# cheolwanpark/tiny-raytracer

Measured on AMD Instinct MI355X. Metric: Mray/s (primary+secondary), higher is better.
Workload: dtype f32; 1 GPU; cornell 2048x2048, depth 50, 256 spp per step (of 4096), streamed, reference-order BVH, seed 1; rays=160658711950, samples=22548578304, image_rows_per_gpu=2048, tuning=default, parallelism=single GPU, world_size=1, launched_by=plain

## Files before the change

### bindings/rust/tinyrt-sys/src/lib.rs

```rust
#![allow(non_camel_case_types)]

use std::os::raw::{c_char, c_int, c_void};

pub const TRT_ABI_VERSION: u32 = 4;

pub const TRT_OK: c_int = 0;
pub const TRT_ERR_INVALID_ARG: c_int = -1;
pub const TRT_ERR_DUPLICATE: c_int = -2;
pub const TRT_ERR_NOT_FOUND: c_int = -3;
pub const TRT_ERR_HIP: c_int = -4;
pub const TRT_ERR_NO_DEVICE: c_int = -5;
pub const TRT_ERR_OOM: c_int = -6;

pub const TRT_LAMBERTIAN: u32 = 0;
pub const TRT_METAL: u32 = 1;
pub const TRT_DIELECTRIC: u32 = 2;
pub const TRT_LIGHT: u32 = 3;

pub const TRT_BACKEND_MEGAKERNEL: u32 = 0;
pub const TRT_BACKEND_WAVEFRONT: u32 = 1;
pub const TRT_BACKEND_AUTO: u32 = 2;
pub const TRT_BACKEND_STREAMED: u32 = 3;

#[repr(C)]
// ... 601 lines not shown
    pub fn trt_denoise_color_default(out: *mut trt_denoise_color);
    pub fn trt_denoise_ex(input: *const trt_denoise_inputs, color: *const trt_denoise_color, width: u32, height: u32,
                          params: *const trt_denoise_params, out: *mut f32) -> c_int;
    pub fn trt_denoise_ex_device(d_in: *const trt_denoise_inputs, color: *const trt_denoise_color, width: u32, height: u32,
                                 params: *const trt_denoise_params, d_out: *mut f32, d_scratch: *mut c_void, scratch_bytes: u64,
                                 stream: *mut c_void) -> c_int;
    pub fn trt_tonemap_u8(accum: *const f32, npixels: u32, gamma: f32, rgb: *mut u8) -> c_int;
    pub fn trt_tonemap_u8_device(d_accum: *const f32, npixels: u32, gamma: f32, d_rgb: *mut u8, stream: *mut c_void) -> c_int;
    pub fn trt_streamed_chunk_spp(width: u32, rows: u32) -> u32;
    pub fn trt_kernel_timing_begin() -> c_int;
    pub fn trt_kernel_timing_end(total_ms: *mut f64, launches: *mut u32) -> c_int;

    pub fn trt_dominant_kernel(s: *const trt_scene, cam: *const trt_camera, p: *const trt_render_params) -> *const c_char;
    pub fn trt_flat_literal_compilations() -> u64;
    pub fn trt_flat_literal_diagnostic() -> *const c_char;

    pub fn trt_last_error() -> *const c_char;
    pub fn trt_device_count() -> c_int;
    pub fn trt_set_device(ordinal: c_int) -> c_int;
    pub fn trt_abi_version() -> u32;
}
```

### include/tinyrt.h

```cpp
#ifndef TINYRT_H
#define TINYRT_H

#include <stddef.h>
#include <stdint.h>

#ifdef __cplusplus
extern "C" {
#endif

#define TRT_ABI_VERSION 4

enum trt_status {
    TRT_OK = 0,
    TRT_ERR_INVALID_ARG = -1,
    TRT_ERR_DUPLICATE = -2,
    TRT_ERR_NOT_FOUND = -3,
    TRT_ERR_HIP = -4,
    TRT_ERR_NO_DEVICE = -5,
    TRT_ERR_OOM = -6
};

typedef struct { float x, y, z; } trt_vec3;
typedef struct { trt_vec3 origin, direction; } trt_ray;
typedef struct { uint32_t x, y; trt_ray ray; } trt_sample_point;
// ... 441 lines not shown
    uint32_t chunk_spp;
    uint32_t dual_walk;
    uint64_t workspace_bytes;
} trt_launch_plan;
int trt_streamed_launch_plan(const trt_scene *s, const trt_camera *cam, const trt_render_params *p, trt_launch_plan *out);

uint32_t trt_streamed_chunk_spp(uint32_t width, uint32_t rows);

int trt_kernel_timing_begin(void);
int trt_kernel_timing_end(double *total_ms, uint32_t *launches);

const char *trt_dominant_kernel(const trt_scene *s, const trt_camera *cam, const trt_render_params *p);

uint64_t trt_flat_literal_compilations(void);
const char *trt_flat_literal_diagnostic(void);

const char *trt_last_error(void);
int trt_device_count(void);
int trt_set_device(int ordinal);
uint32_t trt_abi_version(void);

#ifdef __cplusplus
}
#endif
#endif
```

### tiny-raytracer_amd/_lib.py

```python
import ctypes as C
import os
import subprocess

_HERE = os.path.dirname(os.path.abspath(__file__))
LIB_PATH = os.environ.get("TRT_LIB_PATH") or os.path.join(_HERE, "libtinyrt.so")
CSRC = os.path.join(_HERE, "csrc")

TRT_OK = 0
ABI_VERSION = 4
ERR_INVALID_ARG, ERR_DUPLICATE, ERR_NOT_FOUND, ERR_HIP, ERR_NO_DEVICE, ERR_OOM = -1, -2, -3, -4, -5, -6
LAMBERTIAN, METAL, DIELECTRIC, LIGHT = 0, 1, 2, 3
BACKEND_MEGAKERNEL, BACKEND_WAVEFRONT, BACKEND_AUTO, BACKEND_STREAMED = 0, 1, 2, 3


class Vec3(C.Structure):
    _fields_ = [("x", C.c_float), ("y", C.c_float), ("z", C.c_float)]

    def __init__(self, x=0.0, y=0.0, z=0.0):
        super().__init__(float(x), float(y), float(z))

    def tolist(self):
        return [self.x, self.y, self.z]


# ... 342 lines not shown
                                     C.c_uint64, C.c_void_p]),
    "trt_denoise_color_default": (None, [C.POINTER(DenoiseColor)]),
    "trt_denoise_ex": (C.c_int, [C.POINTER(DenoiseInputs), C.POINTER(DenoiseColor), C.c_uint32, C.c_uint32, C.POINTER(DenoiseParams), C.c_void_p]),
    "trt_denoise_ex_device": (C.c_int, [C.POINTER(DenoiseInputs), C.POINTER(DenoiseColor), C.c_uint32, C.c_uint32, C.POINTER(DenoiseParams),
                                        C.c_void_p, C.c_void_p, C.c_uint64, C.c_void_p]),
    "trt_streamed_chunk_spp": (C.c_uint32, [C.c_uint32, C.c_uint32]),
    "trt_tonemap_u8": (C.c_int, [C.c_void_p, C.c_uint32, C.c_float, C.c_void_p]),
    "trt_tonemap_u8_device": (C.c_int, [C.c_void_p, C.c_uint32, C.c_float, C.c_void_p, C.c_void_p]),
    "trt_dominant_kernel": (C.c_char_p, [C.c_void_p, C.POINTER(CameraPOD), C.POINTER(RenderParams)]),
    "trt_last_error": (C.c_char_p, []),
    "trt_device_count": (C.c_int, []),
    "trt_set_device": (C.c_int, [C.c_int]),
    "trt_abi_version": (C.c_uint32, []),
    "trt_flat_literal_compilations": (C.c_uint64, []),
    "trt_flat_literal_diagnostic": (C.c_char_p, []),
}


def build(force=False):
    if force and os.path.exists(LIB_PATH):
        os.remove(LIB_PATH)
    subprocess.run(["make", "-C", CSRC, "--no-print-directory"], check=True)
    return LIB_PATH


def _share_hip_runtime_with_torch():
    import importlib.util
    try:
        spec = importlib.util.find_spec("torch")
    except (ImportError, ValueError):
# ... 39 lines not shown
```

### tiny-raytracer_amd/csrc/capi.hip

```cpp
#include <hip/hip_runtime.h>

#include <math.h>
#include <stdio.h>
#include <stdlib.h>
#include <string.h>

#include <algorithm>
#include <memory>
#include <mutex>
#include <new>
#include <string>
#include <thread>
#include <vector>

#include "axis_quads.h"
#include "nearest_first.h"
#include "flat_reuse.h"
#include "host_stage.h"
#include "kernels.h"
#include "scene.h"
#include "scene_adopt.h"
#include "scene_cache.h"
#include "scene_query.h"
#include "stream_plan.h"

using namespace trt;

struct trt_world {
    World w;
};

namespace trt {
namespace {
std::mutex g_timing_mu;
bool g_timing_on = false;
unsigned g_timing_epoch = 0;
struct TimingPair { hipEvent_t begin, end; int device; };
// ... 25 lines not shown
    if (o.stream != stream || o.device != dev || o.epoch != epoch || hipEventCreate(&ev) != hipSuccess) {
        (void)hipGetLastError();
        (void)hipEventDestroy(o.ev);
        return;
    }
    if (hipEventRecord(ev, stream) != hipSuccess) { (void)hipGetLastError(); (void)hipEventDestroy(ev); (void)hipEventDestroy(o.ev); return; }
    std::lock_guard<std::mutex> lock(g_timing_mu);
    if (g_timing_on && g_timing_epoch == epoch) g_timing_pairs.push_back(TimingPair{o.ev, ev, dev});
    else { (void)hipEventDestroy(o.ev); (void)hipEventDestroy(ev); }
}
}

struct trt_scene {
    SceneHost host;
    FlatReuse flat_reuse{};
    std::vector<uint32_t> geo_index;
    SceneCache cache;
};

namespace {

thread_local std::string g_last_error;

int fail(int code, const std::string& msg) {
    g_last_error = msg;
    return code;
}
int fail_hip(hipError_t e, const char* what) {
    return fail(TRT_ERR_HIP, std::string(what) + ": " + hipGetErrorString(e));
}
// ... 1 lines not shown
    do {                                                     \
        hipError_t e_ = (call);                              \
        if (e_ != hipSuccess) return fail_hip(e_, #call);    \
    } while (0)

struct Defaults {
    trt_tuning tuning;
    trt_scene_options scene;
    bool flat_reuse = true;
    bool axis_quads = true;
    bool nearest_first = true;
    uint32_t flat_literal = 2;
    bool flat_literal_test_fail = false;
    uint32_t flat_literal_pairs = kLiteralIntervalPairs;
    uint32_t flat_literal_planes = kLiteralPlaneRegs;
};
const Defaults& defaults() {
    static const Defaults d = [] {
        Defaults x;
        x.tuning = tuning_builtin();
        x.scene = scene_options_builtin();
        auto env = [](const char* name) -> const char* { const char* e = getenv(name); return (e && *e) ? e : nullptr; };
        auto u32 = [&](const char* name, uint32_t& field) { if (const char* e = env(name)) field = (uint32_t)strtoul(e, nullptr, 10); };
        trt_tuning& t = x.tuning;
        u32("TRT_STREAM_MINW", t.stream_waves_per_simd); u32("TRT_BIG_THREADS", t.stream_big_threads); u32("TRT_STREAM_BATCH_SPP", t.stream_batch_spp);
        u32("TRT_RADIANCE_GB", t.radiance_gb); u32("TRT_LEAF_SLOTS", t.leaf_slots); u32("TRT_LDS_LEAF_STACK", t.lds_leaf_stack);
        u32("TRT_RAY_POOL", t.ray_pool); u32("TRT_STRAGGLERS", t.stragglers); u32("TRT_LDS_STRAGGLERS", t.lds_stragglers);
        u32("TRT_DUAL_WALK", t.dual_walk); u32("TRT_RUNTIME_WALK", t.runtime_walk); u32("TRT_XCD_REMAP", t.xcd_remap);
        u32("TRT_MINW", t.mega_waves_per_simd); u32("TRT_MEGA_THREADS", t.mega_threads); u32("TRT_MINW8", t.mega_global_waves8);
        u32("TRT_WF_MINW", t.wf_waves_per_simd); u32("TRT_WF_SERVE_MIN", t.wf_serve_min);
        trt_scene_options& o = x.scene;
        if (const char* e = env("TRT_CULL_PRUNE")) {
            const float v = (float)atof(e);
            if (v > 0.0f && v <= 1.0f) o.cull_prune = v;
        }
        if (const char* e = env("TRT_FLAT_WALK")) o.flat_walk = atoi(e) ? 1 : 0;
        if (const char* e = env("TRT_FLAT_REUSE")) x.flat_reuse = atoi(e) != 0;
        if (const char* e = env("TRT_AXIS_QUADS")) x.axis_quads = atoi(e) != 0;
        if (const char* e = env("TRT_NEAREST_FIRST")) x.nearest_first = atoi(e) != 0;
        if (const char* e = env("TRT_FLAT_LITERAL")) x.flat_literal = atoi(e) != 0 ? 1u : 0u;
        if (const char* e = env("TRT_FLAT_LITERAL_TEST_FAIL")) x.flat_literal_test_fail = atoi(e) != 0;
        if (const char* e = env("TRT_FLAT_LITERAL_PAIRS")) { const int v = atoi(e); if (v >= 3 && v <= 8) x.flat_literal_pairs = (uint32_t)v; }
        if (const char* e = env("TRT_FLAT_LITERAL_PLANES")) { const int v = atoi(e); if (v >= 0 && v <= 8 && *e >= '0' && *e <= '9') x.flat_literal_planes = (uint32_t)v; }
        if (const char* e = env("TRT_COMPACT_NODES")) o.compact_nodes = atoi(e) ? 1 : 0;
        if (const char* e = env("TRT_SCRATCH_CAP_MB")) o.scratch_cap_bytes = (uint64_t)strtoull(e, nullptr, 10) << 20;
        return x;
    }();
    return d;
}

[[maybe_unused]] const bool g_defaults_read_at_load = (defaults(), true);

int require_device() {
    int n = 0;
    hipError_t e = hipGetDeviceCount(&n);
    if (e != hipSuccess || n <= 0) {
        (void)hipGetLastError();
        return fail(TRT_ERR_NO_DEVICE, "no HIP device visible: libtinyrt has no CPU path, it needs a gfx950 GPU");
// ... 117 lines not shown
            s->cache.set_short_samples(dev, (rc == TRT_OK && samples < wanted) ? samples : 0u);
        }
        if (rc != TRT_OK) return rc;
        LiteralRequest lit;
        const SceneLayout& L = s->host.layout;
        if (streamed && defaults().flat_literal != 0u && L.flat_walk != 0u && L.n_leaves > 0u &&
            s->host.blob.size() >= 16u * ((size_t)L.off_leaf_list + 2u * (size_t)L.n_leaves)) {
            lit.slot = s->cache.literal_kernel(dev);
            lit.leaf_list = s->host.blob.data() + 16u * (size_t)L.off_leaf_list;
            lit.n_leaves = L.n_leaves;
            const uint64_t call_samples = (uint64_t)cam->width * rows * (ra.sample_end - ra.sample_begin);
            lit.wanted = defaults().flat_literal == 1u || call_samples >= kLiteralAutoSamples;
            lit.empty_source = defaults().flat_literal_test_fail;
            lit.interval_pairs = defaults().flat_reuse ? defaults().flat_literal_pairs : 3u;
            lit.plane_regs = defaults().flat_reuse ? defaults().flat_literal_planes : 0u;
        }
        const LiteralScope lit_scope(lit.slot ? &lit : nullptr);
        hipError_t le;
        if (streamed && d_moment2) {
            le = launch_moments ? launch_moments(sc, cd, ra, tn, ws->ptr, ws->bytes, d_accum, d_moment2, reinterpret_cast<unsigned long long*>(d_counters),
                                                 p->collect_stats != 0, stream)
                                : hipErrorInvalidDeviceFunction;
        } else if (streamed) {
            le = launch_streamed(sc, cd, ra, tn, ws->ptr, ws->bytes, d_accum, reinterpret_cast<unsigned long long*>(d_counters), p->collect_stats != 0, stream);
        } else {
            le = launch_wavefront(sc, cd, ra, tn, ws->ptr, d_accum, reinterpret_cast<unsigned long long*>(d_counters), p->collect_stats != 0, stream);
        }
        rc = s->cache.workspace_release(dev, ws, stream);
        if (le != hipSuccess) return fail_hip(le, streamed ? "launch_streamed" : "launch_wavefront");
        return rc;
// ... 5 lines not shown
void set_flat_reuse(trt_scene* s) {
    const SceneLayout& L = s->host.layout;
    const size_t end = 16u * ((size_t)L.off_leaf_list + 2u * (size_t)L.n_leaves);
    const bool have = L.flat_walk != 0u && L.n_leaves > 0u && s->host.blob.size() >= end;
    uint32_t m[3];
    flat_reuse_masks(have ? s->host.blob.data() + 16u * (size_t)L.off_leaf_list : nullptr, L.n_leaves, have && defaults().flat_reuse, m);
    const size_t qend = 16u * ((size_t)L.off_quad + 5u * (size_t)L.n_quads);
    const bool have_quads = have && L.n_quads > 0u && s->host.blob.size() >= qend;
    const uint32_t aq = axis_quads_flag(have_quads ? s->host.blob.data() + 16u * (size_t)L.off_quad : nullptr, L.n_quads, L.n_leaves, L.flat_walk != 0u,
                                        scene_mode(L) == 1, defaults().axis_quads);
    float planes[3];
    const uint32_t nf = nearest_first_flag(have ? s->host.blob.data() + 16u * (size_t)L.off_leaf_list : nullptr, L.n_leaves,
                                           have_quads ? s->host.blob.data() + 16u * (size_t)L.off_quad : nullptr, L.n_quads, L.n_spheres, aq,
                                           defaults().nearest_first, planes);
    s->flat_reuse = FlatReuse{m[0], m[1], m[2], aq, nf, planes[0], planes[1], planes[2]};
}

void set_geo_index(trt_scene* s) {
    const SceneLayout& L = s->host.layout;
    const std::vector<int32_t>& geo = s->host.reference.prim_geo;
    s->geo_index.assign((size_t)L.n_spheres + L.n_quads, 0xFFFFFFFFu);
    const size_t end = 16u * ((size_t)L.off_ref_nodes + 2u * (size_t)L.n_nodes);
    if (geo.size() < L.n_nodes || s->host.blob.size() < end) return;
    for (uint32_t i = 0; i < L.n_nodes; i++) {
        if (geo[i] < 0) continue;
        uint32_t link;
        memcpy(&link, s->host.blob.data() + 16u * ((size_t)L.off_ref_nodes + 2u * (size_t)i + 1u) + 12u, 4);
        const size_t slot = (size_t)(link & PRIM_INDEX_MASK) + ((link & PRIM_QUAD_BIT) ? L.n_spheres : 0u);
        if (!(link & NODE_INNER_BIT) && slot < s->geo_index.size()) s->geo_index[slot] = (uint32_t)geo[i];
    }
// ... 194 lines not shown
int trt_scene_get_cull_nodes(const trt_scene* s, float* bbox6, int32_t* prim, int32_t* skip, uint32_t cap) {
    if (!s || !bbox6 || !prim || !skip) return fail(TRT_ERR_INVALID_ARG, "null argument");
    return copy_nodes(s->host.culling, bbox6, prim, skip, cap);
}

int trt_scene_get_compact_nodes(const trt_scene* s, uint32_t* words4, uint32_t cap) {
    if (!s || !words4) return fail(TRT_ERR_INVALID_ARG, "null argument");
    const SceneLayout& L = s->host.layout;
    if (L.off_compact == 0u) return fail(TRT_ERR_NOT_FOUND, "scene has no compact node array (it is walked from LDS)");
    if (cap < L.n_cull_nodes) return fail(TRT_ERR_INVALID_ARG, "buffer too small");
    memcpy(words4, s->host.blob.data() + 16u * (size_t)L.off_compact, 16u * (size_t)L.n_cull_nodes);
    for (uint32_t i = 0; i < L.n_cull_nodes; i++)
        if (!(words4[4u * (size_t)i + 3u] & 0x80000000u)) words4[4u * (size_t)i + 3u] >>= 4;
    return TRT_OK;
}
int trt_scene_get_packed(const trt_scene* s, uint8_t* bytes, uint32_t cap) {
    if (!s || !bytes) return fail(TRT_ERR_INVALID_ARG, "null argument");
    const uint32_t n = s->host.layout.blob_bytes;
    if (cap < n) return fail(TRT_ERR_INVALID_ARG, "cap is smaller than the packed scene (trt_scene_info.device_bytes)");
    memcpy(bytes, s->host.blob.data(), n);
    return TRT_OK;
}
int trt_scene_emitters(const trt_scene* s, trt_emitter* out, uint32_t cap, uint32_t* count) {
    if (!s || !count) return fail(TRT_ERR_INVALID_ARG, "null argument");
    if (cap > 0u && !out) return fail(TRT_ERR_INVALID_ARG, "out is null");
    const SceneLayout& L = s->host.layout;
    const F4* const f4 = reinterpret_cast<const F4*>(s->host.blob.data());
    const uint32_t* const u32 = reinterpret_cast<const uint32_t*>(s->host.blob.data());
    try {
        std::vector<trt_emitter> lights;
// ... 431 lines not shown
```

### tiny-raytracer_amd/csrc/flat_literal_rtc.h

```cpp
#pragma once

#include <dlfcn.h>
#include <stdint.h>

#include <string>
#include <vector>

#include "flat_literal.h"

namespace trt {

struct RtcHeader { const char* name; const char* text; };
inline const std::vector<RtcHeader>& rtc_project_headers() {
    static const std::vector<RtcHeader> h = {
#include "rtc_headers.inc"
    };
    return h;
}
inline const std::vector<RtcHeader>& rtc_system_headers() {
    static const std::vector<RtcHeader> h = {
        {"hip/hip_runtime.h", "#pragma once\n"},
        {"stdint.h", "#pragma once\n"
                     "typedef signed char int8_t; typedef unsigned char uint8_t; typedef short int16_t; typedef unsigned short uint16_t;\n"
                     "typedef int int32_t; typedef unsigned int uint32_t; typedef long int64_t; typedef unsigned long uint64_t;\n"
// ... 36 lines not shown
        auto sym = [&](auto& fn, const char* name) { fn = reinterpret_cast<std::remove_reference_t<decltype(fn)>>(dlsym(h, name)); return fn != nullptr; };
        a.ok = sym(a.create, "hiprtcCreateProgram") && sym(a.destroy, "hiprtcDestroyProgram") && sym(a.add_name, "hiprtcAddNameExpression") &&
               sym(a.compile, "hiprtcCompileProgram") && sym(a.log_size, "hiprtcGetProgramLogSize") && sym(a.log, "hiprtcGetProgramLog") &&
               sym(a.lowered, "hiprtcGetLoweredName") && sym(a.code_size, "hiprtcGetCodeSize") && sym(a.code, "hiprtcGetCode");
        return a;
    }();
    return api;
}

struct FlatLiteralBuild {
    std::vector<char> code;
    std::string kernel;
    std::string log;
};

inline std::string flat_literal_source(const std::string& asm_text, uint32_t extra_operands = 0u) {
    return flat_literal_define("TRT_FLAT_LITERAL_ASM", asm_text) + "#define TRT_FLAT_LITERAL_EXTRA " + std::to_string(extra_operands) +
           "\n#include \"stream_pool.h\"\n";
}

inline bool flat_literal_compile(const std::string& source, int minw, const char* arch, const void* beside, FlatLiteralBuild& out) {
    const HiprtcApi& rtc = hiprtc_api(beside);
    if (!rtc.ok) { out.log = "hiprtc not found"; return false; }
    std::vector<const char*> names, texts;
    for (const auto* set : {&rtc_system_headers(), &rtc_project_headers()})
        for (const RtcHeader& h : *set) { names.push_back(h.name); texts.push_back(h.text); }
    HiprtcApi::Program prog = nullptr;
    if (rtc.create(&prog, source.c_str(), "stream_pool_literal.hip", (int)names.size(), texts.data(), names.data()) != 0) { out.log = "hiprtcCreateProgram failed"; return false; }
    const std::string expr = "&trt::stream_pool_kernel<1, false, " + std::to_string(minw) + ", 256, 2, true>";
    const std::string arch_opt = std::string("--offload-arch=") + arch;
    const char* opts[] = {arch_opt.c_str(), "-O3", "-std=c++17", "-ffp-contract=off", "-fno-fast-math", "-fno-slp-vectorize"};
    int rc = rtc.add_name(prog, expr.c_str());
    if (rc == 0) rc = rtc.compile(prog, (int)(sizeof(opts) / sizeof(opts[0])), opts);
// ... 15 lines not shown
```

### tiny-raytracer_amd/csrc/literal_kernel.h

```cpp
#pragma once

#include <stdint.h>

#include <condition_variable>
#include <mutex>

namespace trt {

struct LiteralKernel {
    enum State { UNTRIED, COMPILING, READY, FAILED };
    std::mutex mu;
    std::condition_variable cv;
    State state = UNTRIED;
    void* module = nullptr;
    void* function = nullptr;
    int minw = 0;
    void (*unload)(void* module) = nullptr;
    void release() {
        if (module && unload) unload(module);
        module = function = nullptr;
        state = UNTRIED;
    }
};

constexpr uint32_t kLiteralIntervalPairs = 8u, kLiteralPlaneRegs = 6u;

struct LiteralRequest {
    LiteralKernel* slot = nullptr;
    const void* leaf_list = nullptr;
    uint32_t n_leaves = 0;
    bool wanted = false;
    bool empty_source = false;
    uint32_t interval_pairs = kLiteralIntervalPairs;
    uint32_t plane_regs = kLiteralPlaneRegs;
};
inline thread_local const LiteralRequest* t_literal_request = nullptr;
class LiteralScope {
  public:
    explicit LiteralScope(const LiteralRequest* r) { t_literal_request = r; }
    LiteralScope(const LiteralScope&) = delete;
    ~LiteralScope() { t_literal_request = nullptr; }
};

constexpr uint64_t kLiteralAutoSamples = 1ull << 26;

}
```

### tiny-raytracer_amd/csrc/rt_path.h

```cpp
#pragma once

#include "axis_quads.h"
#include "nearest_first.h"
#include "kernels.h"
#include "rt_device.h"
#include "stream_plan.h"

namespace trt {

extern __shared__ float4 g_lds[];


template <int MODE>
struct SceneAcc {
    const float4* blob;
    SceneLayout L;
    TRT_DEV float4 f4(uint32_t idx) const { return MODE == MODE_LDS ? g_lds[idx] : blob[idx]; }
    TRT_DEV uint32_t u32(uint32_t idx) const {
        return MODE == MODE_LDS ? reinterpret_cast<const uint32_t*>(g_lds)[idx] : reinterpret_cast<const uint32_t*>(blob)[idx];
    }
    TRT_DEV void node(uint32_t i, float4& a, float4& b) const { a = f4(2u * i); b = f4(2u * i + 1u); }
    TRT_DEV void ref_node(uint32_t i, float4& a, float4& b) const { a = blob[L.off_ref_nodes + 2u * i]; b = blob[L.off_ref_nodes + 2u * i + 1u]; }
    TRT_DEV float4 sphere(uint32_t i) const { return f4(L.off_sphere + i); }
    TRT_DEV float4 quad(uint32_t plane, uint32_t i) const { return f4(L.off_quad + 5u * i + plane); }
    TRT_DEV float4 material(uint32_t i) const { return f4(L.off_material + i); }
// ... 112 lines not shown
        pass = slab_fast(na, nb, ray.o, tr.inv, kTMin, tr.t_best);
    } else {
        sc.ref_node(tr.i, na, nb);
        if (tr.fast) pass = slab_fast(na, nb, ray.o, tr.inv, kTMin, tr.t_best);
        else pass = slab_exact(na, nb, ray.o, tr.inv, kTMin, tr.t_best);
    }
    const uint32_t link = __float_as_uint(nb.w);
    const bool inner = (link & NODE_INNER_BIT) != 0u;
    tr.i = (pass && inner) ? (link & ~NODE_INNER_BIT) : __float_as_uint(nb.z);
    return (pass && !inner) ? link : PRIM_NONE;
}

template <int MODE, bool STATS, bool COLD = false>
TRT_DEV void trav_leaf(const SceneAcc<MODE>& sc, const Ray& ray, Trav& tr, uint32_t leaf, Counters<STATS>& ctr, uint32_t axis_quads = 0u) {
    const uint32_t idx = leaf & PRIM_INDEX_MASK;
    if (axis_quads != 0u && (leaf & PRIM_QUAD_BIT)) {
        if constexpr (STATS) ctr.quad_plane++;
        const float4 q0 = sc.quad(0, idx), q1 = sc.quad(1, idx), q2 = sc.quad(2, idx), q3 = sc.quad(3, idx);
        const V3 nrm = v3(q0.x, q0.y, q0.z);
        const float dir_norm = dot(ray.d, nrm);
        const float t = (q0.w - dot(ray.o, nrm)) / dir_norm;
        const bool in_range = (kTMin <= t) & (t < tr.t_best);
        if constexpr (STATS) { if (in_range) ctr.quad_inside++; }
        const V3 p = ray_at(ray, t) - v3(q1.x, q1.y, q1.z);
        const float planar_x = q2.w * dot(p, v3(q2.x, q2.y, q2.z));
        const float planar_y = q2.w * dot(p, v3(q3.x, q3.y, q3.z));
        if (in_range & (0.0f <= planar_x) & (planar_x < 1.0f) & (0.0f <= planar_y) & (planar_y < 1.0f)) {
            tr.t_best = t;
            tr.prim_best = leaf;
        }
    } else if (leaf & PRIM_QUAD_BIT) {
        if constexpr (STATS) ctr.quad_plane++;
        const float4 q0 = sc.quad(0, idx), q1 = sc.quad(1, idx), q2 = sc.quad(2, idx), q3 = sc.quad(3, idx), q4 = sc.quad(4, idx);
        const V3 nrm = v3(q0.x, q0.y, q0.z);
        const float dir_norm = dot(ray.d, nrm);
        const float t = (q0.w - dot(ray.o, nrm)) / dir_norm;
        const bool in_range = (kTMin <= t) & (t < tr.t_best);
        if constexpr (STATS) { if (in_range) ctr.quad_inside++; }
        const V3 p = ray_at(ray, t) - v3(q1.x, q1.y, q1.z);
        const V3 vv = v3(q2.x, q2.y, q2.z), ww = v3(q2.w, q3.x, q3.y), uu = v3(q3.z, q3.w, q4.x);
        const float planar_x = dot(cross(p, vv), ww);
        const float planar_y = dot(cross(uu, p), ww);
        if (in_range & (0.0f <= planar_x) & (planar_x < 1.0f) & (0.0f <= planar_y) & (planar_y < 1.0f)) {
            tr.t_best = t;
            tr.prim_best = leaf;
        }
// ... 690 lines not shown
template <int MODE, bool STATS, int WALK, bool ANY = false>
TRT_DEV bool closest_hit_resume(const SceneAcc<MODE>& sc, const Ray& ray, Trav& tr, Counters<STATS>& ctr, uint32_t leaf_slots, float2* lds_stack,
                                const float4* __restrict__ leaf_list, const uint4* __restrict__ nodes16, uint32_t stragglers, uint32_t entered) {
    static_assert(WALK == WALK_COMPACT || WALK == WALK_LDS_STACK, "only the per-lane tree walks with an LDS leaf stack can be left and resumed");
    if (__builtin_expect(!tr.ref, 1)) {
        if constexpr (WALK == WALK_COMPACT) return walk_compact<MODE, STATS, ANY>(sc, nodes16, leaf_list, ray, tr, ctr, lds_stack, leaf_slots, stragglers, entered);
        else return walk_fast_lds<MODE, STATS, ANY>(sc, ray, tr, ctr, lds_stack, leaf_slots, stragglers, entered);
    }
    closest_hit_ref<MODE, STATS, ANY>(sc, ray, tr, ctr);
    return true;
}

template <int MODE>
TRT_DEV uint32_t prim_material(const SceneAcc<MODE>& sc, uint32_t prim) {
    const uint32_t idx = prim & PRIM_INDEX_MASK;
    return (prim & PRIM_QUAD_BIT) ? __float_as_uint(sc.quad(1, idx).w) : sc.sphere_material(idx);
}

struct Path {
    Ray ray;
    V3 color, atten;
    uint32_t remain;
    Rng rng;
};

constexpr uint32_t SHADE_KIND_MISS = 0xFFFFFFFFu;
struct ShadeInfo {
    bool hide_light;
    uint32_t kind;
    V3 normal;
};
template <int MODE, bool STATS, bool LAZY, bool INFO>
TRT_DEV bool shade_body(const SceneAcc<MODE>& sc, Path& p, uint32_t prim, float t, V3 background, Counters<STATS>& ctr, ShadeInfo* info) {
    if (prim == PRIM_NONE) {
        p.color = (LAZY ? v3(0.0f, 0.0f, 0.0f) : p.color) + p.atten * background;
        if constexpr (INFO) info->kind = SHADE_KIND_MISS;
        return true;
    }
    if constexpr (STATS) ctr.shade++;
    const uint32_t idx = prim & PRIM_INDEX_MASK;
    V3 point = ray_at(p.ray, t);
    V3 normal;
    bool front_face;
    uint32_t mat;
    if (prim & PRIM_QUAD_BIT) {
        float4 q0 = sc.quad(0, idx), q1 = sc.quad(1, idx), q4 = sc.quad(4, idx);
        front_face = dot(p.ray.d, v3(q0.x, q0.y, q0.z)) < 0.0f;
        V3 nu = v3(q4.y, q4.z, q4.w);
        normal = front_face ? nu : -nu;
        mat = __float_as_uint(q1.w);
    } else {
        float4 sp = sc.sphere(idx);
        V3 outward = point - v3(sp.x, sp.y, sp.z);
        front_face = dot(p.ray.d, outward) < 0.0f;
        V3 nu = normalized(outward);
        normal = front_face ? nu : -nu;
        mat = sc.sphere_material(idx);
    }
    const float4 m = sc.material(mat);
    const uint32_t kind = sc.material_kind(mat);
// ... 41 lines not shown
    } else {
        return true;
    }
    p.atten = p.atten * albedo;
    p.ray = ray_new(point, dir);
    p.remain -= 1u;
    return p.remain == 0u;
}
template <int MODE, bool STATS, bool LAZY = false>
TRT_DEV bool shade_hit(const SceneAcc<MODE>& sc, Path& p, uint32_t prim, float t, V3 background, Counters<STATS>& ctr) {
    return shade_body<MODE, STATS, LAZY, false>(sc, p, prim, t, background, ctr, nullptr);
}
template <int MODE, bool STATS>
TRT_DEV bool shade_hit_info(const SceneAcc<MODE>& sc, Path& p, uint32_t prim, float t, V3 background, Counters<STATS>& ctr, ShadeInfo& info) {
    return shade_body<MODE, STATS, false, true>(sc, p, prim, t, background, ctr, &info);
}

TRT_DEV Ray primary_ray(const CameraDev& cam, uint32_t x, uint32_t y, Rng& rng) {
    const float nu = (float)x + rng_random(rng);
    const float nv = (float)y + rng_random(rng);
    float u, v;
    pixel_uv(cam.width, cam.height, nu, nv, u, v);
    float px, py;
    random_in_unit_disk(rng, px, py);
    V3 pos = v3(cam.pos[0], cam.pos[1], cam.pos[2]);
    V3 du = v3(cam.du[0], cam.du[1], cam.du[2]), dv = v3(cam.dv[0], cam.dv[1], cam.dv[2]);
    V3 origin = (pos + px * du) + py * dv;
    V3 ul = v3(cam.upper_left[0], cam.upper_left[1], cam.upper_left[2]);
    V3 hor = v3(cam.horizontal[0], cam.horizontal[1], cam.horizontal[2]);
    V3 ver = v3(cam.vertical[0], cam.vertical[1], cam.vertical[2]);
// ... 66 lines not shown
```

### tiny-raytracer_amd/csrc/stream_pool.h

```cpp
#pragma once

#include "kernels.h"
#include "rt_path.h"
#include "stream_plan.h"
#include "wave_run.h"

namespace trt {

struct StreamKernargs {
    SceneDev scd; CameraDev cam; RenderArgs ra;
    float* colors; uint32_t* batch_counter; unsigned long long* counters;
    uint32_t tiles_x, n_tiles, n_batches, batch_spp;
    const float4* leaf_list; const uint4* nodes16;
};
struct StreamTileArgs { uint32_t tiles_x, n_tiles, n_batches, batch_spp; };
template <class T>
TRT_DEV T kernarg_reload(size_t offset) {
    static_assert(sizeof(T) % 4 == 0, "whole words");
    typedef const __attribute__((address_space(4))) uint32_t* WordPtr;
    WordPtr w = (WordPtr)__builtin_amdgcn_kernarg_segment_ptr() + offset / 4;
    asm volatile("" : "+s"(w));
    uint32_t words[sizeof(T) / 4];
#pragma unroll
    for (uint32_t i = 0; i < sizeof(T) / 4; i++) words[i] = w[i];
// ... 104 lines not shown
            if constexpr (kResumable) {
                Trav tr = trav_begin<MODE, WALK == WALK_COMPACT>(sc, p.ray, false);
                if (walking) trav_unpark(leaf_stack, tr); else n_rays++;
                const uint32_t entered = (uint32_t)__builtin_popcountll(__builtin_amdgcn_ballot_w64(true));
                walking = !closest_hit_resume<MODE, STATS, WALK>(sc, p.ray, tr, ctr, ra.leaf_slots, leaf_stack, leaf_list, nodes16, ra.stragglers, entered);
                if (!walking) {
                    if (shade_hit<MODE, STATS, LAZY>(sc, p, tr.prim_best, tr.t_best, background, ctr)) {
                        radiance_store(kernarg_reload<float*>(offsetof(StreamKernargs, colors)), out_idx, p.color);
                        has_path = false;
                    }
                }
            } else {
                n_rays++;
                float t;
                const uint32_t prim = closest_hit<MODE, STATS, WALK>(sc, p.ray, STATS && ra.ref_tree != 0u, t, ctr, ra.leaf_slots, leaf_stack, leaf_list, nodes16, flat_reuse);
                if (shade_hit<MODE, STATS, LAZY>(sc, p, prim, t, background, ctr)) {
                    radiance_store(kernarg_reload<float*>(offsetof(StreamKernargs, colors)), out_idx, p.color);
                    has_path = false;
                }
            }
        }
        TRT_CLK(ctr, 3);
    }
    flush_counters<STATS>(counters, n_samples, n_rays, ctr);
}

}
```

### tiny-raytracer_amd/csrc/streamed.hip

```cpp
#include <mutex>
#include <string>

#include "flat_literal_rtc.h"
#include "host_stage.h"
#include "kernels.h"
#include "literal_kernel.h"
#include "rt_path.h"
#include "stream_plan.h"
#include "stream_pool.h"
#include "wave_run.h"

namespace trt {

template <int MODE, bool STATS, int MINW = 1, int THREADS = 256, int WALK = WALK_RUNTIME, bool LAZY = false>
__global__ __launch_bounds__(THREADS, MINW) void stream_sample_kernel(SceneDev scd, CameraDev cam, RenderArgs ra,
                                                                             float* __restrict__ colors,
                                                                             uint32_t* __restrict__ batch_counter,
                                                                             unsigned long long* __restrict__ counters,
                                                                             uint32_t tiles_x, uint32_t n_tiles, uint32_t n_batches, uint32_t batch_spp,
                                                                             const float4* __restrict__ leaf_list,
                                                                             const uint4* __restrict__ nodes16) {
    stage_scene_to_lds<MODE>(scd);
    const FlatReuse flat_reuse = axis_quads_to_lds<MODE, STATS, WALK>(scd, ra.flat_reuse);
    const SceneAcc<MODE> sc{scd.blob, scd.L};
// ... 315 lines not shown
#define TRT_FN_POOL(MODE, STATS, MINW, THREADS, WALK, LAZY) reinterpret_cast<const void*>(&stream_pool_kernel<MODE, STATS, MINW, THREADS, WALK, LAZY>),
#define TRT_FN_SAMPLE(MODE, STATS, MINW, THREADS, WALK, LAZY) reinterpret_cast<const void*>(&stream_sample_kernel<MODE, STATS, MINW, THREADS, WALK, LAZY>),
#define TRT_FN_DUAL(MINW) reinterpret_cast<const void*>(&stream_dual_kernel<MINW, 256>),
const void* const kStreamKernelFns[] = {
    TRT_STREAM_SPECIALISED(TRT_FN_POOL, TRT_FN_SAMPLE, TRT_FN_DUAL)
    TRT_STREAM_GENERAL(TRT_FN_POOL, TRT_FN_SAMPLE, TRT_FN_DUAL)
};
#undef TRT_FN_POOL
#undef TRT_FN_SAMPLE
#undef TRT_FN_DUAL
static_assert(sizeof(kStreamKernelFns) / sizeof(kStreamKernelFns[0]) == kStreamKernelCount, "one address per shape row");

std::mutex g_literal_mu;
unsigned long long g_literal_compilations = 0;
std::string g_literal_diagnostic;
thread_local std::string t_literal_diagnostic_copy;

void literal_unload(void* module) {
    (void)hipModuleUnload(static_cast<hipModule_t>(module));
    (void)hipGetLastError();
}

bool literal_build(LiteralKernel& slot, const LiteralRequest& rq, const FlatReuse& reuse, int minw, std::string& why) {
    {
        std::lock_guard<std::mutex> lock(g_literal_mu);
        g_literal_compilations++;
    }
    int dev = 0;
    hipDeviceProp_t prop;
    if (hipGetDevice(&dev) != hipSuccess || hipGetDeviceProperties(&prop, dev) != hipSuccess) { (void)hipGetLastError(); why = "no device properties"; return false; }
    std::string arch(prop.gcnArchName);
    arch = arch.substr(0, arch.find(':'));
    const uint32_t masks[3] = {reuse.x, reuse.y, reuse.z};
    std::string text, source;
    if (!rq.empty_source) {
        FlatCacheStats cache;
        if (!flat_literal_cached_asm(rq.leaf_list, rq.n_leaves, masks, rq.interval_pairs, rq.plane_regs, text, cache)) { why = "leaf list refused"; return false; }
        source = flat_literal_source(text, cache.extra_operands);
    }
    FlatLiteralBuild built;
    if (!flat_literal_compile(source, minw, arch.c_str(), reinterpret_cast<const void*>(&hipModuleLoadData), built)) { why = "hiprtc: " + built.log; return false; }
    hipModule_t mod = nullptr;
    hipFunction_t fn = nullptr;
    hipError_t e = hipModuleLoadData(&mod, built.code.data());
    if (e == hipSuccess) e = hipModuleGetFunction(&fn, mod, built.kernel.c_str());
    if (e != hipSuccess) {
        (void)hipGetLastError();
        if (mod) (void)hipModuleUnload(mod);
        why = std::string("module load: ") + hipGetErrorString(e);
        return false;
    }
    slot.module = mod; slot.function = fn; slot.minw = minw; slot.unload = &literal_unload;
    return true;
}

hipFunction_t literal_kernel_for(const StreamLaunchPlan& pl, const RenderArgs& ra, bool stats) {
    const LiteralRequest* rq = t_literal_request;
#ifdef TRT_PHASE_CLOCK
    return nullptr;
#endif
    if (!kAsmBoxLoop) return nullptr;
    if (!rq || !rq->slot || stats || !pl.specialised || !pl.pool || pl.dual || pl.walk != WALK_FLAT || pl.mode != MODE_LDS || ra.ref_tree ||
        pl.kernel_walk != WALK_FLAT || pl.threads != 256 || pl.lds_bytes > 48u * 1024u || rq->n_leaves > kFlatLiteralMaxLeaves) return nullptr;
    LiteralKernel& slot = *rq->slot;
    std::unique_lock<std::mutex> lock(slot.mu);
    while (slot.state == LiteralKernel::COMPILING) slot.cv.wait(lock);
    if (slot.state == LiteralKernel::UNTRIED && rq->wanted) {
        slot.state = LiteralKernel::COMPILING;
        lock.unlock();
        std::string why;
        const bool ok = literal_build(slot, *rq, ra.flat_reuse, pl.kernel_minw, why);
        if (!ok) {
            std::lock_guard<std::mutex> g(g_literal_mu);
            g_literal_diagnostic = "lock-step kernel not compiled for its scene, the built-in kernel runs: " + why;
        }
        lock.lock();
        slot.state = ok ? LiteralKernel::READY : LiteralKernel::FAILED;
        slot.cv.notify_all();
    }
    if (slot.state != LiteralKernel::READY || slot.minw != pl.kernel_minw) return nullptr;
    return static_cast<hipFunction_t>(slot.function);
}

}

static hipError_t launch_streamed_folds(const SceneDev& sc, const CameraDev& cam, const RenderArgs& ra_all, const trt_tuning& tn, void* workspace, size_t workspace_bytes,
                                        float* d_accum, float* d_moment2, unsigned long long* d_counters, bool stats, hipStream_t stream) {
    if (ra_all.rows_local == 0 || cam.width == 0) return hipSuccess;
    uint32_t* batch_counter = static_cast<uint32_t*>(workspace);
    float* colors = reinterpret_cast<float*>(static_cast<char*>(workspace) + kWorkspaceHeader);
    const uint32_t samples_all = ra_all.sample_end - ra_all.sample_begin;
    uint32_t chunk_full = streamed_chunk_spp(cam.width, ra_all.rows_local, tn.radiance_gb);
    const uint32_t granted = streamed_chunk_that_fits(cam.width, ra_all.rows_local, workspace_bytes);
    if (granted == 0u) return hipErrorInvalidValue;
    if (chunk_full > granted) chunk_full = granted;
// ... 88 lines not shown

int trt_variance_device(const float* d_accum, const float* d_moment2, uint32_t npixels, uint32_t samples_per_pixel, float* d_variance, void* stream) {
    if (npixels && (!d_accum || !d_moment2 || !d_variance)) return trt::query_fail(TRT_ERR_INVALID_ARG, "null argument");
    if (npixels == 0u) return TRT_OK;
    const int rc = trt::query_require_device();
    if (rc != TRT_OK) return rc;
    const hipError_t e = trt::launch_variance(d_accum, d_moment2, npixels, samples_per_pixel, d_variance, static_cast<hipStream_t>(stream));
    if (e != hipSuccess) return trt::query_fail_hip(e, "variance launch");
    return TRT_OK;
}

uint64_t trt_flat_literal_compilations(void) {
    std::lock_guard<std::mutex> lock(trt::g_literal_mu);
    return trt::g_literal_compilations;
}
const char* trt_flat_literal_diagnostic(void) {
    std::lock_guard<std::mutex> lock(trt::g_literal_mu);
    trt::t_literal_diagnostic_copy = trt::g_literal_diagnostic;
    return trt::t_literal_diagnostic_copy.c_str();
}

int trt_variance(const float* accum, const float* moment2, uint32_t npixels, uint32_t samples_per_pixel, float* variance) {
    return trt::host_form([&]() -> int {
        if (npixels && (!accum || !moment2 || !variance)) return trt::query_fail(TRT_ERR_INVALID_ARG, "null argument");
        if (npixels == 0u) return TRT_OK;
        const int rc = trt::query_require_device();
        if (rc != TRT_OK) return rc;
        const size_t frame = (size_t)npixels * 12u;
        trt::HostStage st("variance buffers");
        const size_t r_s = st.reserve(frame), r_m = st.reserve(frame), r_v = st.reserve((size_t)npixels * 4u);
// ... 11 lines not shown
```

Baseline: 78530 Mray/s.

## Specialise runtime-compiled kernel on derived scene facts (quads only, material kinds)

Derives per-scene facts on the host (all primitives are quads, which material kinds occur, whether the lazy colour path applies) and passes them as preprocessor defines into the hiprtc-compiled lock-step kernel. With those defines the traversal and shading drop the sphere branches, and for quad-only Lambertian/light scenes a straight-line shade function replaces the general shade_hit. This is meant to cut branches, divergence and register pressure in the hot loop, at the cost of a more specialised kernel and a cache key that now includes the facts. Correctness depends on the derivation matching the scene; Cornell has only quads with Lambertian and light materials.

```diff
diff --git a/bindings/rust/tinyrt-sys/src/lib.rs b/bindings/rust/tinyrt-sys/src/lib.rs
--- a/bindings/rust/tinyrt-sys/src/lib.rs
+++ b/bindings/rust/tinyrt-sys/src/lib.rs
@@ -639,6 +639,8 @@
     pub fn trt_dominant_kernel(s: *const trt_scene, cam: *const trt_camera, p: *const trt_render_params) -> *const c_char;
     pub fn trt_flat_literal_compilations() -> u64;
     pub fn trt_flat_literal_diagnostic() -> *const c_char;
+    pub fn trt_scene_facts(s: *const trt_scene) -> u32;
+    pub fn trt_flat_literal_facts() -> u32;
 
     pub fn trt_last_error() -> *const c_char;
     pub fn trt_device_count() -> c_int;
diff --git a/include/tinyrt.h b/include/tinyrt.h
--- a/include/tinyrt.h
+++ b/include/tinyrt.h
@@ -479,6 +479,8 @@
 
 uint64_t trt_flat_literal_compilations(void);
 const char *trt_flat_literal_diagnostic(void);
+uint32_t trt_scene_facts(const trt_scene *s);
+uint32_t trt_flat_literal_facts(void);
 
 const char *trt_last_error(void);
 int trt_device_count(void);
diff --git a/tiny-raytracer_amd/_lib.py b/tiny-raytracer_amd/_lib.py
--- a/tiny-raytracer_amd/_lib.py
+++ b/tiny-raytracer_amd/_lib.py
@@ -380,6 +380,8 @@
     "trt_abi_version": (C.c_uint32, []),
     "trt_flat_literal_compilations": (C.c_uint64, []),
     "trt_flat_literal_diagnostic": (C.c_char_p, []),
+    "trt_scene_facts": (C.c_uint32, [C.c_void_p]),
+    "trt_flat_literal_facts": (C.c_uint32, []),
 }
 
 
diff --git a/tiny-raytracer_amd/csrc/capi.hip b/tiny-raytracer_amd/csrc/capi.hip
--- a/tiny-raytracer_amd/csrc/capi.hip
+++ b/tiny-raytracer_amd/csrc/capi.hip
@@ -21,6 +21,7 @@
 #include "scene.h"
 #include "scene_adopt.h"
 #include "scene_cache.h"
+#include "scene_facts.h"
 #include "scene_query.h"
 #include "stream_plan.h"
 
@@ -76,6 +77,7 @@
 struct trt_scene {
     SceneHost host;
     FlatReuse flat_reuse{};
+    SceneFacts facts;
     std::vector<uint32_t> geo_index;
     SceneCache cache;
 };
@@ -107,6 +109,7 @@
     bool flat_literal_test_fail = false;
     uint32_t flat_literal_pairs = kLiteralIntervalPairs;
     uint32_t flat_literal_planes = kLiteralPlaneRegs;
+    uint32_t scene_facts = SCENE_FACTS_ALL;
 };
 const Defaults& defaults() {
     static const Defaults d = [] {
@@ -135,6 +138,12 @@
         if (const char* e = env("TRT_FLAT_LITERAL_TEST_FAIL")) x.flat_literal_test_fail = atoi(e) != 0;
         if (const char* e = env("TRT_FLAT_LITERAL_PAIRS")) { const int v = atoi(e); if (v >= 3 && v <= 8) x.flat_literal_pairs = (uint32_t)v; }
         if (const char* e = env("TRT_FLAT_LITERAL_PLANES")) { const int v = atoi(e); if (v >= 0 && v <= 8 && *e >= '0' && *e <= '9') x.flat_literal_planes = (uint32_t)v; }
+        if (const char* e = env("TRT_SCENE_FACTS")) {
+            char* end = nullptr;
+            const long v = strtol(e, &end, 10);
+            const bool number = end != e && *end == '\0';
+            x.scene_facts = (number && v == 0) ? SCENE_FACTS_NONE : (number && v == 1) ? SCENE_FACTS_CONSTANTS : SCENE_FACTS_ALL;
+        }
         if (const char* e = env("TRT_COMPACT_NODES")) o.compact_nodes = atoi(e) ? 1 : 0;
         if (const char* e = env("TRT_SCRATCH_CAP_MB")) o.scratch_cap_bytes = (uint64_t)strtoull(e, nullptr, 10) << 20;
         return x;
@@ -282,6 +291,7 @@
             lit.empty_source = defaults().flat_literal_test_fail;
             lit.interval_pairs = defaults().flat_reuse ? defaults().flat_literal_pairs : 3u;
             lit.plane_regs = defaults().flat_reuse ? defaults().flat_literal_planes : 0u;
+            lit.facts = s->facts;
         }
         const LiteralScope lit_scope(lit.slot ? &lit : nullptr);
         hipError_t le;
@@ -317,6 +327,14 @@
                                            have_quads ? s->host.blob.data() + 16u * (size_t)L.off_quad : nullptr, L.n_quads, L.n_spheres, aq,
                                            defaults().nearest_first, planes);
     s->flat_reuse = FlatReuse{m[0], m[1], m[2], aq, nf, planes[0], planes[1], planes[2]};
+    const size_t kend = 4u * ((size_t)L.off_material_kind + L.n_materials), smend = 4u * ((size_t)L.off_sphere_mat + L.n_spheres);
+    const bool have_mats = have && s->host.blob.size() >= kend && s->host.blob.size() >= smend && (L.n_quads == 0u || have_quads);
+    s->facts = have_mats ? scene_facts_derive(s->host.blob.data() + 16u * (size_t)L.off_leaf_list, L.n_leaves,
+                                              have_quads ? s->host.blob.data() + 16u * (size_t)L.off_quad : nullptr, L.n_quads, L.n_spheres,
+                                              reinterpret_cast<const uint32_t*>(s->host.blob.data()) + L.off_sphere_mat,
+                                              reinterpret_cast<const uint32_t*>(s->host.blob.data()) + L.off_material_kind, L.n_materials, aq, nf,
+                                              L.lazy_color, defaults().scene_facts)
+                           : SceneFacts{};
 }
 
 void set_geo_index(trt_scene* s) {
@@ -541,6 +559,8 @@
         if (!(words4[4u * (size_t)i + 3u] & 0x80000000u)) words4[4u * (size_t)i + 3u] >>= 4;
     return TRT_OK;
 }
+uint32_t trt_scene_facts(const trt_scene* s) { return s ? s->facts.word() : 0u; }
+
 int trt_scene_get_packed(const trt_scene* s, uint8_t* bytes, uint32_t cap) {
     if (!s || !bytes) return fail(TRT_ERR_INVALID_ARG, "null argument");
     const uint32_t n = s->host.layout.blob_bytes;
diff --git a/tiny-raytracer_amd/csrc/flat_literal_rtc.h b/tiny-raytracer_amd/csrc/flat_literal_rtc.h
--- a/tiny-raytracer_amd/csrc/flat_literal_rtc.h
+++ b/tiny-raytracer_amd/csrc/flat_literal_rtc.h
@@ -7,6 +7,7 @@
 #include <vector>
 
 #include "flat_literal.h"
+#include "scene_facts.h"
 
 namespace trt {
 
@@ -74,9 +75,9 @@
     std::string log;
 };
 
-inline std::string flat_literal_source(const std::string& asm_text, uint32_t extra_operands = 0u) {
-    return flat_literal_define("TRT_FLAT_LITERAL_ASM", asm_text) + "#define TRT_FLAT_LITERAL_EXTRA " + std::to_string(extra_operands) +
-           "\n#include \"stream_pool.h\"\n";
+inline std::string flat_literal_source(const std::string& asm_text, uint32_t extra_operands = 0u, const SceneFacts& facts = SceneFacts{}) {
+    return flat_literal_define("TRT_FLAT_LITERAL_ASM", asm_text) + "#define TRT_FLAT_LITERAL_EXTRA " + std::to_string(extra_operands) + "\n" +
+           scene_facts_defines(facts) + "#include \"stream_pool.h\"\n";
 }
 
 inline bool flat_literal_compile(const std::string& source, int minw, const char* arch, const void* beside, FlatLiteralBuild& out) {
diff --git a/tiny-raytracer_amd/csrc/literal_kernel.h b/tiny-raytracer_amd/csrc/literal_kernel.h
--- a/tiny-raytracer_amd/csrc/literal_kernel.h
+++ b/tiny-raytracer_amd/csrc/literal_kernel.h
@@ -4,6 +4,8 @@
 
 #include <condition_variable>
 #include <mutex>
+
+#include "scene_facts.h"
 
 namespace trt {
 
@@ -15,6 +17,7 @@
     void* module = nullptr;
     void* function = nullptr;
     int minw = 0;
+    SceneFacts facts;
     void (*unload)(void* module) = nullptr;
     void release() {
         if (module && unload) unload(module);
@@ -33,6 +36,7 @@
     bool empty_source = false;
     uint32_t interval_pairs = kLiteralIntervalPairs;
     uint32_t plane_regs = kLiteralPlaneRegs;
+    SceneFacts facts;
 };
 inline thread_local const LiteralRequest* t_literal_request = nullptr;
 class LiteralScope {
diff --git a/tiny-raytracer_amd/csrc/rt_path.h b/tiny-raytracer_amd/csrc/rt_path.h
--- a/tiny-raytracer_amd/csrc/rt_path.h
+++ b/tiny-raytracer_amd/csrc/rt_path.h
@@ -9,6 +9,20 @@
 namespace trt {
 
 extern __shared__ float4 g_lds[];
+
+#ifndef TRT_FACT_NO_SPHERE
+#define TRT_FACT_NO_SPHERE 0
+#endif
+#ifndef TRT_FACT_KINDS
+#define TRT_FACT_KINDS 0
+#endif
+#ifndef TRT_FACT_STRAIGHT_SHADE
+#define TRT_FACT_STRAIGHT_SHADE 0
+#endif
+constexpr bool kFactNoSphere = TRT_FACT_NO_SPHERE != 0;
+constexpr uint32_t kFactKinds = TRT_FACT_KINDS;
+constexpr bool kFactStraightShade = kFactNoSphere && TRT_FACT_STRAIGHT_SHADE != 0;
+constexpr bool fact_kind_possible(uint32_t kind) { return kFactKinds == 0u || ((kFactKinds >> kind) & 1u) != 0u; }
 
 
 template <int MODE>
@@ -151,7 +165,7 @@
 template <int MODE, bool STATS, bool COLD = false>
 TRT_DEV void trav_leaf(const SceneAcc<MODE>& sc, const Ray& ray, Trav& tr, uint32_t leaf, Counters<STATS>& ctr, uint32_t axis_quads = 0u) {
     const uint32_t idx = leaf & PRIM_INDEX_MASK;
-    if (axis_quads != 0u && (leaf & PRIM_QUAD_BIT)) {
+    if (axis_quads != 0u && (kFactNoSphere || (leaf & PRIM_QUAD_BIT))) {
         if constexpr (STATS) ctr.quad_plane++;
         const float4 q0 = sc.quad(0, idx), q1 = sc.quad(1, idx), q2 = sc.quad(2, idx), q3 = sc.quad(3, idx);
         const V3 nrm = v3(q0.x, q0.y, q0.z);
@@ -166,7 +180,7 @@
             tr.t_best = t;
             tr.prim_best = leaf;
         }
-    } else if (leaf & PRIM_QUAD_BIT) {
+    } else if (kFactNoSphere || (leaf & PRIM_QUAD_BIT)) {
         if constexpr (STATS) ctr.quad_plane++;
         const float4 q0 = sc.quad(0, idx), q1 = sc.quad(1, idx), q2 = sc.quad(2, idx), q3 = sc.quad(3, idx), q4 = sc.quad(4, idx);
         const V3 nrm = v3(q0.x, q0.y, q0.z);
@@ -887,7 +901,7 @@
 template <int MODE>
 TRT_DEV uint32_t prim_material(const SceneAcc<MODE>& sc, uint32_t prim) {
     const uint32_t idx = prim & PRIM_INDEX_MASK;
-    return (prim & PRIM_QUAD_BIT) ? __float_as_uint(sc.quad(1, idx).w) : sc.sphere_material(idx);
+    return (kFactNoSphere || (prim & PRIM_QUAD_BIT)) ? __float_as_uint(sc.quad(1, idx).w) : sc.sphere_material(idx);
 }
 
 struct Path {
@@ -916,7 +930,7 @@
     V3 normal;
     bool front_face;
     uint32_t mat;
-    if (prim & PRIM_QUAD_BIT) {
+    if (kFactNoSphere || (prim & PRIM_QUAD_BIT)) {
         float4 q0 = sc.quad(0, idx), q1 = sc.quad(1, idx), q4 = sc.quad(4, idx);
         front_face = dot(p.ray.d, v3(q0.x, q0.y, q0.z)) < 0.0f;
         V3 nu = v3(q4.y, q4.z, q4.w);
@@ -988,6 +1002,36 @@
 template <int MODE, bool STATS>
 TRT_DEV bool shade_hit_info(const SceneAcc<MODE>& sc, Path& p, uint32_t prim, float t, V3 background, Counters<STATS>& ctr, ShadeInfo& info) {
     return shade_body<MODE, STATS, false, true>(sc, p, prim, t, background, ctr, &info);
+}
+
+template <int MODE>
+TRT_DEV bool shade_straight(const SceneAcc<MODE>& sc, Path& p, uint32_t prim, float t, V3 background) {
+    const bool miss = prim == PRIM_NONE;
+    static_assert(!kFactStraightShade || kFactNoSphere, "the straight-line shade is claimed for scenes of quads only (scene_facts.h)");
+    const uint32_t idx = miss ? 0u : (prim & PRIM_INDEX_MASK);
+    const V3 point = ray_at(p.ray, t);
+    const float4 q0 = sc.quad(0, idx), q1 = sc.quad(1, idx), q4 = sc.quad(4, idx);
+    const bool front_face = dot(p.ray.d, v3(q0.x, q0.y, q0.z)) < 0.0f;
+    const V3 nu = v3(q4.y, q4.z, q4.w);
+    const V3 normal = front_face ? nu : -nu;
+    const uint32_t mat = __float_as_uint(q1.w);
+    const float4 m = sc.material(mat);
+    const bool light = fact_kind_possible(TRT_LIGHT) && sc.material_kind(mat) == TRT_LIGHT;
+    const V3 in_sphere = random_in_unit_sphere_unit(p.rng);
+    V3 dir = normal + normalized(in_sphere);
+    if (near_zero(dir)) dir = normal;
+    const V3 factor = miss ? background : v3(m.x, m.y, m.z);
+    p.atten = p.atten * factor;
+    V3 origin = point;
+    asm volatile("" : "+v"(origin.x), "+v"(origin.y), "+v"(origin.z), "+v"(dir.x), "+v"(dir.y), "+v"(dir.z));
+    p.ray = ray_new(origin, dir);
+    p.remain -= 1u;
+    const bool lit = miss | light;
+    const bool ended = lit | (p.remain == 0u);
+    V3 c = v3(__builtin_nondeterministic_value(0.0f), __builtin_nondeterministic_value(0.0f), __builtin_nondeterministic_value(0.0f));
+    if (ended) c = lit ? v3(0.0f, 0.0f, 0.0f) + p.atten : v3(0.0f, 0.0f, 0.0f);
+    p.color = c;
+    return ended;
 }
 
 TRT_DEV Ray primary_ray(const CameraDev& cam, uint32_t x, uint32_t y, Rng& rng) {
diff --git a/tiny-raytracer_amd/csrc/scene_facts.h b/tiny-raytracer_amd/csrc/scene_facts.h
--- /dev/null
+++ b/tiny-raytracer_amd/csrc/scene_facts.h
@@ -0,0 +1,76 @@
+#pragma once
+
+#include <stdint.h>
+#include <stdio.h>
+#include <string.h>
+
+#include <string>
+
+namespace trt {
+
+struct SceneFacts {
+    bool no_sphere = false;
+    uint32_t kinds = 0u;
+    bool axis_exact = false;
+    bool nearest_first = false;
+    bool lazy_color = false;
+    bool straight_shade = false;
+    bool any() const { return no_sphere || kinds != 0u || axis_exact || nearest_first || lazy_color || straight_shade; }
+    bool operator==(const SceneFacts& o) const {
+        return no_sphere == o.no_sphere && kinds == o.kinds && axis_exact == o.axis_exact && nearest_first == o.nearest_first &&
+               lazy_color == o.lazy_color && straight_shade == o.straight_shade;
+    }
+    bool operator!=(const SceneFacts& o) const { return !(*this == o); }
+    uint32_t word() const {
+        return (no_sphere ? 1u : 0u) | (axis_exact ? 2u : 0u) | (nearest_first ? 4u : 0u) | (lazy_color ? 8u : 0u) | (straight_shade ? 16u : 0u) | (kinds << 8);
+    }
+};
+
+constexpr uint32_t kFactKindCount = 4u;
+constexpr uint32_t kFactMaxLeaves = 32u;
+
+enum : uint32_t { SCENE_FACTS_NONE = 0u, SCENE_FACTS_CONSTANTS = 1u, SCENE_FACTS_ALL = 2u };
+
+inline SceneFacts scene_facts_derive(const void* leaf_list, uint32_t n_leaves, const void* quads, uint32_t n_quads, uint32_t n_spheres,
+                                     const uint32_t* sphere_material, const uint32_t* material_kind, uint32_t n_materials, uint32_t axis_quads,
+                                     uint32_t nearest_first, uint32_t lazy_color, uint32_t level = SCENE_FACTS_ALL) {
+    SceneFacts f;
+    if (level == SCENE_FACTS_NONE || leaf_list == nullptr || n_leaves == 0u || n_leaves > kFactMaxLeaves || material_kind == nullptr) return f;
+    if ((uint64_t)n_quads + n_spheres != n_leaves) return f;
+    const unsigned char* lp = static_cast<const unsigned char*>(leaf_list);
+    bool all_quads = n_spheres == 0u;
+    uint32_t kinds = 0u;
+    for (uint32_t i = 0; i < n_leaves; i++) {
+        uint32_t link, mat;
+        memcpy(&link, lp + 32u * (size_t)i + 28u, sizeof link);
+        const uint32_t idx = link & 0x3FFFFFFFu;
+        if (link & 0x80000000u) return SceneFacts{};
+        if (link & 0x40000000u) {
+            if (quads == nullptr || idx >= n_quads) return SceneFacts{};
+            memcpy(&mat, static_cast<const unsigned char*>(quads) + 80u * (size_t)idx + 28u, sizeof mat);
+        } else {
+            all_quads = false;
+            if (sphere_material == nullptr || idx >= n_spheres) return SceneFacts{};
+            mat = sphere_material[idx];
+        }
+        if (mat >= n_materials || material_kind[mat] >= kFactKindCount) return SceneFacts{};
+        kinds |= 1u << material_kind[mat];
+    }
+    f.no_sphere = all_quads;
+    f.kinds = kinds;
+    f.axis_exact = f.no_sphere && axis_quads != 0u;
+    f.nearest_first = f.axis_exact && nearest_first != 0u;
+    f.lazy_color = lazy_color != 0u;
+    f.straight_shade = level >= SCENE_FACTS_ALL && f.no_sphere && f.lazy_color && (kinds & ~((1u << 0) | (1u << 3))) == 0u;
+    return f;
+}
+
+inline std::string scene_facts_defines(const SceneFacts& f) {
+    std::string s;
+    if (f.no_sphere) s += "#define TRT_FACT_NO_SPHERE 1\n";
+    if (f.kinds != 0u) { char b[48]; snprintf(b, sizeof b, "#define TRT_FACT_KINDS 0x%x\n", f.kinds); s += b; }
+    if (f.straight_shade) s += "#define TRT_FACT_STRAIGHT_SHADE 1\n";
+    return s;
+}
+
+}
diff --git a/tiny-raytracer_amd/csrc/stream_pool.h b/tiny-raytracer_amd/csrc/stream_pool.h
--- a/tiny-raytracer_amd/csrc/stream_pool.h
+++ b/tiny-raytracer_amd/csrc/stream_pool.h
@@ -142,7 +142,10 @@
                 n_rays++;
                 float t;
                 const uint32_t prim = closest_hit<MODE, STATS, WALK>(sc, p.ray, STATS && ra.ref_tree != 0u, t, ctr, ra.leaf_slots, leaf_stack, leaf_list, nodes16, flat_reuse);
-                if (shade_hit<MODE, STATS, LAZY>(sc, p, prim, t, background, ctr)) {
+                bool ended;
+                if constexpr (kFactStraightShade && !STATS && LAZY) ended = shade_straight<MODE>(sc, p, prim, t, background);
+                else ended = shade_hit<MODE, STATS, LAZY>(sc, p, prim, t, background, ctr);
+                if (ended) {
                     radiance_store(kernarg_reload<float*>(offsetof(StreamKernargs, colors)), out_idx, p.color);
                     has_path = false;
                 }
diff --git a/tiny-raytracer_amd/csrc/streamed.hip b/tiny-raytracer_amd/csrc/streamed.hip
--- a/tiny-raytracer_amd/csrc/streamed.hip
+++ b/tiny-raytracer_amd/csrc/streamed.hip
@@ -353,6 +353,7 @@
 std::mutex g_literal_mu;
 unsigned long long g_literal_compilations = 0;
 std::string g_literal_diagnostic;
+uint32_t g_literal_facts_word = 0;
 thread_local std::string t_literal_diagnostic_copy;
 
 void literal_unload(void* module) {
@@ -372,10 +373,11 @@
     arch = arch.substr(0, arch.find(':'));
     const uint32_t masks[3] = {reuse.x, reuse.y, reuse.z};
     std::string text, source;
+    const SceneFacts unit_facts = rq.empty_source ? SceneFacts{} : rq.facts;
     if (!rq.empty_source) {
         FlatCacheStats cache;
         if (!flat_literal_cached_asm(rq.leaf_list, rq.n_leaves, masks, rq.interval_pairs, rq.plane_regs, text, cache)) { why = "leaf list refused"; return false; }
-        source = flat_literal_source(text, cache.extra_operands);
+        source = flat_literal_source(text, cache.extra_operands, unit_facts);
     }
     FlatLiteralBuild built;
     if (!flat_literal_compile(source, minw, arch.c_str(), reinterpret_cast<const void*>(&hipModuleLoadData), built)) { why = "hiprtc: " + built.log; return false; }
@@ -389,7 +391,11 @@
         why = std::string("module load: ") + hipGetErrorString(e);
         return false;
     }
-    slot.module = mod; slot.function = fn; slot.minw = minw; slot.unload = &literal_unload;
+    slot.module = mod; slot.function = fn; slot.minw = minw; slot.facts = unit_facts; slot.unload = &literal_unload;
+    {
+        std::lock_guard<std::mutex> lock(g_literal_mu);
+        g_literal_facts_word = unit_facts.word();
+    }
     return true;
 }
 
@@ -417,7 +423,7 @@
         slot.state = ok ? LiteralKernel::READY : LiteralKernel::FAILED;
         slot.cv.notify_all();
     }
-    if (slot.state != LiteralKernel::READY || slot.minw != pl.kernel_minw) return nullptr;
+    if (slot.state != LiteralKernel::READY || slot.minw != pl.kernel_minw || slot.facts != rq->facts) return nullptr;
     return static_cast<hipFunction_t>(slot.function);
 }
 
@@ -536,6 +542,10 @@
     std::lock_guard<std::mutex> lock(trt::g_literal_mu);
     return trt::g_literal_compilations;
 }
+uint32_t trt_flat_literal_facts(void) {
+    std::lock_guard<std::mutex> lock(trt::g_literal_mu);
+    return trt::g_literal_facts_word;
+}
 const char* trt_flat_literal_diagnostic(void) {
     std::lock_guard<std::mutex> lock(trt::g_literal_mu);
     trt::t_literal_diagnostic_copy = trt::g_literal_diagnostic;
```

Result: faster. 81790 Mray/s, median of 6 (+4.2%).
